# rhuangr/MARL-Maze

Measured on AMD Instinct MI355X. Metric: env-steps/sec (2-agent 10x10 maze) + PPO updates/sec, higher is better.
Workload: dtype f32; 1 GPU; PPO rollout+GAE+update over 65536 parallel 10x10 2-agent mazes per GPU (configs[2], the north-star workload: 65,536 parallel 10x10 mazes per GPU); mazes_per_gpu=65536, maze=10x10 (layout 19x19), horizon=16, global_batch=1048575, minibatch=209715, minibatch_steps_per_iter=25, parallelism=dp1, rollout=stream launches, gemm=x2, parity_mode=True

## Files before the change

include/marlmaze.h:

```cpp
#ifndef MARLMAZE_H
#define MARLMAZE_H

#include <stdint.h>

#ifdef __cplusplus
extern "C" {
#endif

#define MM_OBS_DIM 65
#define MM_MASK_DIM 6
#define MM_RNG_WORDS 625
#define MM_MAX_SIDE 41
#define MM_MAZES_PER_BLOCK 32

#define MM_E_ARG (-1)
#define MM_E_SIZE (-2)

#define MM_ST_GEN_FAIL 1u
#define MM_ST_BAD_MOVE 2u

typedef struct {
    int8_t x, y, dir, flags;
    int8_t lmx, lmy, olsx, olsy;
    int8_t minx, maxx, miny, maxy;
// ... 250 lines not shown
int mm_par_accum(const uint8_t* done, const float* reward, const int32_t* ep_stats, const int32_t* par, int n,
                 int quota, int32_t* counted, uint64_t* totals, void* stream);

#define MM_ELOG_WORDS 16
#define MM_ELOG_LEN 0
#define MM_ELOG_SHORTEST 1
#define MM_ELOG_SOLVED 2
#define MM_ELOG_PAR 3
#define MM_ELOG_T_KEY 4
#define MM_ELOG_FETCHER 5
#define MM_ELOG_T_KNOW0 6
#define MM_ELOG_T_KNOW1 7
#define MM_ELOG_T_READY 8
#define MM_ELOG_CELLS0 9
#define MM_ELOG_CELLS1 10
#define MM_ELOG_CELLS_BOTH 11
#define MM_ELOG_OPEN 12
#define MM_ELOG_MARKS0 13
#define MM_ELOG_MARKS1 14
#define MM_ELOG_STAYS 15
long mm_elog_state_words(int layout_stride);
int mm_elog_init(int32_t* log, int32_t* counted, int32_t* state, int n, int quota, long state_words, void* stream);
int mm_elog_start(const mm_env_t* env, const uint8_t* select, int32_t* state, long state_words, void* stream);
int mm_elog_step(const mm_env_t* env, const int8_t* actions, const uint8_t* done, const float* reward,
                 const int32_t* ep_stats, const int32_t* par, int quota, int32_t* counted, int32_t* state,
                 long state_words, int32_t* log, void* stream);

int mm_critic_value(const float* x, int ldx, int K0, int M, int H0, int H1, const float* w0, const float* b0,
                    const float* w1, const float* b1, const float* w2, const float* b2, float* v, void* stream);

int mm_critic_update_ok(int M, int K0, int ldx);
int mm_critic_update(const float* x, int ldx, int K0, int M, const float* rtg, const uint16_t* w0_tp, const float* b0,
                     const uint16_t* w1_tp, const uint16_t* w1t_tp, const float* b1, const uint16_t* w2_tp,
                     const float* w2, const float* b2, float* v, float* dv, float* h0, float* h1, float* dy1,
                     float* dy0, float* cs1, float* cs0, void* stream);

int mm_actor_front_ws_len(void);
int mm_actor_front_prep(const float* const* wproj, const float* const* bproj, const float* wq, const float* wk,
                        const float* wv, float* ws, void* stream);
int mm_actor_front_fwd(const float* ws, const float* x, int ldx, int B, int parity, float* h, void* stream);

#define MM_FRONT_FWD_ROW1 0
#define MM_FRONT_FWD_ROW2 1
#define MM_FRONT_FWD_MFMA 2
int mm_actor_front_fwd_ex(const float* ws, const float* x, int ldx, int B, int parity, float* h, int algo,
                          void* stream);

int mm_actor_front_grad_len(void);
int mm_actor_front_partial_len(void);
int mm_actor_front_bwd(const float* ws, const float* x, int ldx, int B, int parity, const float* dh, float* partial,
                       int grid, float* red, float* grad, void* stream);
#define MM_FRONT_BWD_MFMA 0
#define MM_FRONT_BWD_VALU 1
int mm_actor_front_bwd_ex(const float* ws, const float* x, int ldx, int B, int parity, const float* dh,
                          float* partial, int grid, float* red, float* grad, int algo, void* stream);
int mm_actor_front_bwd_grid(int B, int algo);
int mm_actor_front_bwd_to(const float* ws, const float* x, int ldx, int B, int parity, const float* dh,
                          float* partial, int grid, float* red, float* const* wproj_grad, float* const* bproj_grad,
                          float* wq_grad, float* wk_grad, float* wv_grad, int algo, void* stream);

#ifdef __cplusplus
}
#endif
#endif
```

marl-maze_amd/csrc/actor_front.hip:

```cpp
#include <hip/hip_runtime.h>
#include <math.h>
#include <stdint.h>

#include "marlmaze.h"

namespace mm {

#ifndef FRONT_P3_UNROLL
#define FRONT_P3_UNROLL 4
#endif
#ifndef FRONT_EF_UNROLL
#define FRONT_EF_UNROLL 2
#endif
#ifndef FRONT_EF_ROWS
#define FRONT_EF_ROWS 4
#endif

constexpr int kTok = 23;
constexpr int kEmb = 20;
constexpr int kKq = 10;
constexpr int kQkv = 2 * kKq + kEmb;
constexpr int kPin = 4;
constexpr int kRowF = kTok * kEmb;
constexpr float kSqrtKq = 3.16227766016838f;
// ... 1342 lines not shown
            for (int I = 0; I < 2; I++)
                if (16 * I + c16 < 24)
#pragma unroll
                    for (int J = 0; J < 2; J++)
                        t_store(T + (16 * I + c16) * kTp + 16 * J + 4 * q4, dS[J][I], t_sw(c16));
            wave_sync();
            f32x4_t dK[2] = {f32x4_t{0.f, 0.f, 0.f, 0.f}, f32x4_t{0.f, 0.f, 0.f, 0.f}};
            f32x4_t dQ[2] = {f32x4_t{0.f, 0.f, 0.f, 0.f}, f32x4_t{0.f, 0.f, 0.f, 0.f}};
#pragma unroll
            for (int s = 0; s < kKH; s++) {
                const int i = kh_row(s, q4);
#pragma unroll
                for (int J = 0; J < 2; J++) dK[J] = mfma4(T[i * kTp + 16 * J + t_col(s, c16, q4)], qb[s], dK[J]);
#pragma unroll
                for (int I = 0; I < 2; I++) {
                    const int rb = (16 * I + c16) * kTp;
                    const float tv = s < 4 ? T[(rb + 4 * q4 + t_sw(c16)) ^ s] : T[rb + 16 + 4 * (s - 4) + (q4 ^ t_sw(c16))];
                    dQ[I] = mfma4(ka[s], tv, dQ[I]);
                }
            }
            front_prio(2);
            wave_sync();
#pragma unroll
            for (int I = 0; I < 2; I++) {
                const int i = 16 * I + c16;
                if (i < kTok && q4 < 3)
                    *reinterpret_cast<float4*>(my + kMG + i * kQkv + 4 * q4) =
                        make_float4(dQ[I][0], dQ[I][1], dQ[I][2], dQ[I][3]);
            }
#pragma unroll
            for (int J = 0; J < 2; J++)
#pragma unroll
                for (int g = 0; g < 4; g++) {
                    const int j = 16 * J + 4 * q4 + g;
                    if (j < kTok) {
                        if (c16 < kKq) my[kMG + j * kQkv + kKq + c16] = dK[J][g];
#pragma unroll
                        for (int C = 0; C < 2; C++)
                            if (16 * C + c16 < kEmb) my[kMG + j * kQkv + 2 * kKq + 16 * C + c16] = dV[J][C][g];
                    }
                }
        }
        float4 fp[kEFPf];
        ef2_prefetch(dh + (size_t)row0 * kRowF, nrow, 0, fp);
        if (hs < nrow && tok < kTok) *reinterpret_cast<float4*>(sm + hs * kMSample + kMX + tok * kPin) = xv;
        __syncthreads();
#ifndef FRONT_DIAG_NO_EF
        ef2_accumulate<kMSample, kMG, kMX>(sm, dh + (size_t)row0 * kRowF, nrow, fp, ef);
#endif
    }
    ef2_write(partial, ef);
}

constexpr int kSumCols = 64, kSumClasses = 16;

__global__ __launch_bounds__(kSumCols * kSumClasses) void k_front_sum(const float* __restrict__ partial, int rows,
                                                                      double* __restrict__ red) {
    __shared__ double acc_s[kSumClasses][kSumCols];
    const int c = threadIdx.x % kSumCols, k = threadIdx.x / kSumCols;
    const int e = blockIdx.x * kSumCols + c;
    double acc = 0.0;
    if (e < kPartLen) {
        int r = k;
        for (; r + 7 * kSumClasses < rows; r += 8 * kSumClasses) {
            float v[8];
#pragma unroll
            for (int i = 0; i < 8; i++) v[i] = partial[(size_t)(r + i * kSumClasses) * kPartLen + e];
#pragma unroll
            for (int i = 0; i < 8; i++) acc += (double)v[i];
        }
        for (; r < rows; r += kSumClasses) acc += (double)partial[(size_t)r * kPartLen + e];
    }
    acc_s[k][c] = acc;
    __syncthreads();
    if (k == 0 && e < kPartLen) {
        double t = 0.0;
#pragma unroll
        for (int q = 0; q < kSumClasses; q++) t += acc_s[q][c];
        red[e] = t;
    }
}

struct FrontGradPtrs {
    float* wq;
    float* wk;
    float* wv;
    float* wp[kTok];
    float* bp[kTok];
};

template <bool SCATTER>
__global__ __launch_bounds__(256) void k_front_combine(const float* __restrict__ ws, const double* __restrict__ red,
                                                       float* __restrict__ grad, FrontGradPtrs dst) {
    const int e = blockIdx.x * blockDim.x + threadIdx.x;
    if (e >= kGradLen) return;
    auto put = [&](double vd) {
        const float v = (float)vd;
        if (!SCATTER) {
            grad[e] = v;
        } else if (e < kGP) {
            const int r = e / kEmb, c = e % kEmb;
            float* d = r < kKq ? dst.wq + r * kEmb : r < 2 * kKq ? dst.wk + (r - kKq) * kEmb : dst.wv + (r - 2 * kKq) * kEmb;
            d[c] = v;
        } else if (e < kGB) {
            const int f = e - kGP, tk = f / (kEmb * kPin), c = (f / kPin) % kEmb, k = f % kPin;
            if (k < c_dims[tk]) dst.wp[tk][c * c_dims[tk] + k] = v;
        } else {
            const int f = e - kGB;
            dst.bp[f / kEmb][f % kEmb] = v;
        }
    };
    const float* W = ws + kWsW;
    if (e < kGP) {
        const int r = e / kEmb, c = e % kEmb;
        double acc = 0.0;
        for (int tk = 0; tk < kTok; tk++) {
            const float* Wp = ws + kWsWP + (tk * kEmb + c) * kPin;
            const double* E = red + kPEF + (tk * kGd + r) * kPin;
#pragma unroll
            for (int a = 0; a < kPin; a++) acc = fma(E[a], (double)Wp[a], acc);
            acc = fma(red[kPef + tk * kGd + r], (double)ws[kWsBP + tk * kEmb + c], acc);
        }
        put(acc);
    } else if (e < kGB) {
        const int f = e - kGP, tk = f / (kEmb * kPin), c = (f / kPin) % kEmb, k = f % kPin;
        double acc = red[kPEF + (tk * kGd + kQkv + c) * kPin + k];
        for (int r = 0; r < kQkv; r++) acc = fma((double)W[r * kEmb + c], red[kPEF + (tk * kGd + r) * kPin + k], acc);
        put(acc);
    } else {
        const int f = e - kGB, tk = f / kEmb, c = f % kEmb;
        double acc = red[kPef + tk * kGd + kQkv + c];
        for (int r = 0; r < kQkv; r++) acc = fma((double)W[r * kEmb + c], red[kPef + tk * kGd + r], acc);
        put(acc);
    }
}

}

using namespace mm;

extern "C" int mm_actor_front_ws_len(void) { return kWsLen; }
extern "C" int mm_actor_front_grad_len(void) { return kGradLen; }
static int cu_count() {
    static int cus[64] = {0};
    int dev = 0;
    if (hipGetDevice(&dev) != hipSuccess || dev < 0 || dev >= 64) return 256;
    if (!cus[dev] && hipDeviceGetAttribute(&cus[dev], hipDeviceAttributeMultiprocessorCount, dev) != hipSuccess)
        cus[dev] = 256;
    return cus[dev];
}

extern "C" int mm_actor_front_partial_len(void) { return kPartLen; }

extern "C" int mm_actor_front_bwd_grid(int B, int algo) {
    if (B < 0 || (algo != MM_FRONT_BWD_MFMA && algo != MM_FRONT_BWD_VALU)) return MM_E_ARG;
    const int rows = algo == MM_FRONT_BWD_MFMA ? kMRows : kBwdRows;
    const int per_cu = algo == MM_FRONT_BWD_MFMA ? kMPerCU : 2;
    const int groups = (B + rows - 1) / rows;
    const int cap = per_cu * cu_count();
    return groups < 1 ? 1 : (groups < cap ? groups : cap);
}

extern "C" int mm_actor_front_prep(const float* const* wproj, const float* const* bproj, const float* wq,
                                   const float* wk, const float* wv, float* ws, void* stream) {
    if (!wproj || !bproj || !wq || !wk || !wv || !ws) return MM_E_ARG;
    ProjPtrs P;
    for (int i = 0; i < kTok; i++) {
        if (!wproj[i] || !bproj[i]) return MM_E_ARG;
        P.w[i] = wproj[i];
        P.b[i] = bproj[i];
    }
    hipLaunchKernelGGL(k_front_prep, dim3(kTok), dim3(256), 0, (hipStream_t)stream, P, wq, wk, wv, ws);
    return (int)hipGetLastError();
}


extern "C" int mm_actor_front_fwd_ex(const float* ws, const float* x, int ldx, int B, int parity, float* h,
                                     int algo, void* stream) {
    if (!ws || !x || !h || B < 0 || ldx < MM_OBS_DIM) return MM_E_ARG;
    if (algo != MM_FRONT_FWD_ROW1 && algo != MM_FRONT_FWD_ROW2 && algo != MM_FRONT_FWD_MFMA) return MM_E_ARG;
    if (B == 0) return 0;
    if (algo == MM_FRONT_FWD_MFMA) {
        const int groups = (B + kFMRows - 1) / kFMRows;
        const int cap = FRONT_FM_WAVES * cu_count();
        const int grid = groups < cap ? groups : cap;
        hipLaunchKernelGGL(k_front_fwd_mfma<false>, dim3(grid), dim3(256), 0, (hipStream_t)stream, ws, x, ldx, B,
                           parity, (void*)h);
    } else if (algo == MM_FRONT_FWD_ROW2) {
        const int groups = (B + kF2Rows - 1) / kF2Rows;
        const int grid = groups < 2 * cu_count() ? groups : 2 * cu_count();
        hipLaunchKernelGGL(k_front_fwd2, dim3(grid), dim3(256), 0, (hipStream_t)stream, ws, x, ldx, B, parity, h);
    } else {
        const int groups = (B + kFwdRows - 1) / kFwdRows;
        const int grid = groups < 3 * cu_count() ? groups : 3 * cu_count();
        hipLaunchKernelGGL(k_front_fwd<false>, dim3(grid), dim3(256), 0, (hipStream_t)stream, ws, x, ldx, B, parity,
                           (void*)h);
    }
    return (int)hipGetLastError();
}

extern "C" int mm_actor_front_fwd_h16_ex(const float* ws, const float* x, int ldx, int B, int parity, void* h,
                                         int algo, void* stream) {
    if (!ws || !x || !h || B < 0 || ldx < MM_OBS_DIM || ((uintptr_t)h & 7)) return MM_E_ARG;
    if (algo != MM_FRONT_FWD_ROW1 && algo != MM_FRONT_FWD_MFMA) return MM_E_ARG;
    if (B == 0) return 0;
    if (algo == MM_FRONT_FWD_MFMA) {
        const int groups = (B + kFMRows - 1) / kFMRows;
        const int cap = FRONT_FM_WAVES * cu_count();
        const int grid = groups < cap ? groups : cap;
        hipLaunchKernelGGL(k_front_fwd_mfma<true>, dim3(grid), dim3(256), 0, (hipStream_t)stream, ws, x, ldx, B,
                           parity, h);
    } else {
        const int groups = (B + kFwdRows - 1) / kFwdRows;
        const int grid = groups < 3 * cu_count() ? groups : 3 * cu_count();
        hipLaunchKernelGGL(k_front_fwd<true>, dim3(grid), dim3(256), 0, (hipStream_t)stream, ws, x, ldx, B, parity,
                           h);
    }
    return (int)hipGetLastError();
}

extern "C" int mm_actor_front_fwd_h16(const float* ws, const float* x, int ldx, int B, int parity, void* h,
                                      void* stream) {
    return mm_actor_front_fwd_h16_ex(ws, x, ldx, B, parity, h, MM_FRONT_FWD_ROW1, stream);
}

extern "C" int mm_actor_front_fwd(const float* ws, const float* x, int ldx, int B, int parity, float* h,
                                  void* stream) {
    return mm_actor_front_fwd_ex(ws, x, ldx, B, parity, h, MM_FRONT_FWD_ROW1, stream);
}

static int front_bwd(const float* ws, const float* x, int ldx, int B, int parity, const float* dh, float* partial,
                     int grid, float* red, float* grad, const FrontGradPtrs* dst, int algo, void* stream) {
    if (!ws || !x || !dh || !partial || !red || (!grad && !dst) || B < 0 || ldx < MM_OBS_DIM || grid <= 0)
        return MM_E_ARG;
    if ((uintptr_t)red & 7) return MM_E_ARG;
    if (algo != MM_FRONT_BWD_MFMA && algo != MM_FRONT_BWD_VALU) return MM_E_ARG;
    hipStream_t s = (hipStream_t)stream;
    double* red64 = reinterpret_cast<double*>(red);
    if (algo == MM_FRONT_BWD_MFMA)
        hipLaunchKernelGGL(k_front_bwd_mfma, dim3(grid), dim3(kMThreads), 0, s, ws, x, ldx, B, parity, dh, partial);
    else
        hipLaunchKernelGGL(k_front_bwd, dim3(grid), dim3(kBwdThreads), 0, s, ws, x, ldx, B, parity, dh, partial);
    hipError_t e = hipGetLastError();
    if (e != hipSuccess) return (int)e;
    hipLaunchKernelGGL(k_front_sum, dim3((kPartLen + kSumCols - 1) / kSumCols), dim3(kSumCols * kSumClasses), 0, s,
                       partial, grid, red64);
    e = hipGetLastError();
    if (e != hipSuccess) return (int)e;
    if (grad)
        hipLaunchKernelGGL(k_front_combine<false>, dim3((kGradLen + 255) / 256), dim3(256), 0, s, ws, red64, grad,
                           FrontGradPtrs{});
    else
        hipLaunchKernelGGL(k_front_combine<true>, dim3((kGradLen + 255) / 256), dim3(256), 0, s, ws, red64, nullptr, *dst);
    return (int)hipGetLastError();
}

extern "C" int mm_actor_front_bwd_ex(const float* ws, const float* x, int ldx, int B, int parity, const float* dh,
                                     float* partial, int grid, float* red, float* grad, int algo, void* stream) {
    if (!grad) return MM_E_ARG;
    return front_bwd(ws, x, ldx, B, parity, dh, partial, grid, red, grad, nullptr, algo, stream);
}

extern "C" int mm_actor_front_bwd_to(const float* ws, const float* x, int ldx, int B, int parity, const float* dh,
                                     float* partial, int grid, float* red, float* const* wproj_grad,
                                     float* const* bproj_grad, float* wq_grad, float* wk_grad, float* wv_grad,
                                     int algo, void* stream) {
    if (!wproj_grad || !bproj_grad || !wq_grad || !wk_grad || !wv_grad) return MM_E_ARG;
    FrontGradPtrs d;
    d.wq = wq_grad;
    d.wk = wk_grad;
    d.wv = wv_grad;
    for (int i = 0; i < kTok; i++) {
        if (!wproj_grad[i] || !bproj_grad[i]) return MM_E_ARG;
        d.wp[i] = wproj_grad[i];
        d.bp[i] = bproj_grad[i];
    }
    return front_bwd(ws, x, ldx, B, parity, dh, partial, grid, red, nullptr, &d, algo, stream);
}

extern "C" int mm_actor_front_bwd(const float* ws, const float* x, int ldx, int B, int parity, const float* dh,
                                  float* partial, int grid, float* red, float* grad, void* stream) {
    return mm_actor_front_bwd_ex(ws, x, ldx, B, parity, dh, partial, grid, red, grad, MM_FRONT_BWD_VALU, stream);
}
```

marl-maze_amd/marlmaze/_lib.py:

```python
import ctypes
import os

import torch

PKG_ROOT = os.path.dirname(os.path.dirname(os.path.abspath(__file__)))
LIB_PATH = os.environ.get("MARLMAZE_LIB") or os.path.join(PKG_ROOT, "libmarlmaze.so")

OBS_DIM = 65
MASK_DIM = 6
RNG_WORDS = 625
MAX_SIDE = 41
MAZES_PER_BLOCK = 32

ST_GEN_FAIL = 1
ST_BAD_MOVE = 2

GAE_AUTO, GAE_COLUMN, GAE_WALK, GAE_SCAN = 0, 1, 2, 3

ACT_SAMPLE, ACT_GREEDY = 0, 1
ACT_MODES = {"sample": ACT_SAMPLE, "greedy": ACT_GREEDY}

EVAL_WORDS = 32
EV_EPISODES, EV_SOLVED, EV_TIMEOUTS, EV_SUM_LEN, EV_SUM_LEN_SOLVED, EV_SUM_SHORT_SOLVED = 0, 1, 2, 3, 4, 5
EV_MIN_LEN_SOLVED, EV_MAX_LEN_SOLVED, EV_SUM_RATIO_Q16, EV_BAD_SHORT = 6, 7, 8, 9
EV_HIST0, EV_HIST_BINS = 16, 16

PAR_WORDS = 32
PAR_EPISODES, PAR_SUM_LEN, PAR_SUM_PAR, PAR_SUM_RATIO_Q16, PAR_AT_PAR, PAR_BELOW = 0, 1, 2, 3, 4, 5
PAR_UNRATED, PAR_MAX_EXCESS = 6, 7
PAR_HIST0, PAR_HIST_BINS = 16, 16

ELOG_WORDS = 16
ELOG_LEN, ELOG_SHORTEST, ELOG_SOLVED, ELOG_PAR, ELOG_T_KEY, ELOG_FETCHER, ELOG_T_KNOW0, ELOG_T_KNOW1 = range(8)
ELOG_T_READY, ELOG_CELLS0, ELOG_CELLS1, ELOG_CELLS_BOTH, ELOG_OPEN, ELOG_MARKS0, ELOG_MARKS1, ELOG_STAYS = range(8, 16)
ELOG_FIELDS = ("LEN", "SHORTEST", "SOLVED", "PAR", "T_KEY", "FETCHER", "T_KNOW0", "T_KNOW1", "T_READY", "CELLS0",
               "CELLS1", "CELLS_BOTH", "OPEN", "MARKS0", "MARKS1", "STAYS")

AF_KNOWS_END = 1
AF_SEES_END = 2
AF_OTHER_KNOWS = 4
AF_HAS_KEY = 8
AF_SEES_KEY = 16
AF_TEAM_KEY = 32
AF_HAS_MARK = 64

EXPORTS = ("mm_version", "mm_env_desc_size", "mm_layout_stride", "mm_env_seed", "mm_env_reset",
           "mm_env_step", "mm_env_step_timed", "mm_env_reset_done", "mm_env_pregen", "mm_gae", "mm_gae_ex", "mm_sample", "mm_head_sample", "mm_head_sample_ex", "mm_heads_fwd",
           "mm_actor_front_ws_len", "mm_actor_front_prep", "mm_actor_front_fwd", "mm_actor_front_fwd_ex",
           "mm_actor_front_grad_len", "mm_actor_front_partial_len", "mm_actor_front_bwd", "mm_actor_front_bwd_ex",
           "mm_actor_front_bwd_to", "mm_actor_front_bwd_grid",
           "mm_x3_tp_len", "mm_x3_tp_pack", "mm_x3_nt", "mm_x3_nt_f32a", "mm_x3_mbits_len",
           "mm_x3_heads_bwd", "mm_ppo_loss_partials", "mm_ppo_loss", "mm_ppo_loss_bwd",
           "mm_gemm_tp_len", "mm_gemm_tp_pack", "mm_gemm_nt", "mm_gemm_nt_algo", "mm_gemm_wgrad_algo", "mm_gemm_wgrad_ws_len",
           "mm_gemm_wgrad", "mm_colsum", "mm_mse_loss_partials", "mm_mse_loss", "mm_losses_final",
           "mm_clip_adam_ws_len", "mm_clip_adam", "mm_gemm_tp_pack_multi", "mm_gemm_wgrad_slices",
           "mm_gemm_wgrad_partials", "mm_colsum_multi_ws_len", "mm_colsum_multi", "mm_wsum_multi", "mm_critic_value",
           "mm_gemm_range_flag", "mm_gemm_nt_h", "mm_gemm_a16_ok", "mm_gemm_wgrad_h", "mm_gemm_wgrad_partials_h",
           "mm_heads_fwd_h16", "mm_x3_heads_bwd_h16", "mm_trunk3_ok", "mm_trunk3",
           "mm_trunk3_head_sample_ok", "mm_trunk3_head_sample", "mm_actor_front_fwd_h16",
           "mm_actor_front_fwd_h16_ex", "mm_head_act", "mm_act", "mm_eval_init", "mm_eval_accum",
           "mm_env_dist", "mm_env_par", "mm_par_init", "mm_par_accum",
           "mm_elog_state_words", "mm_elog_init", "mm_elog_start", "mm_elog_step",
           "mm_gemm_x2p_ok", "mm_x3_heads_bwd_x2p",
           "mm_critic_update_ok", "mm_critic_update")
VERSION = 308

PREC_X3, PREC_F16, PREC_X2 = 0, 1, 2
FRONT_BWD = {"mfma": 0, "valu": 1}
FRONT_FWD = {"row1": 0, "row2": 1, "mfma": 2}
GEMM_ALGO = {"auto": 0, "stream": 1}
GEMM_A_F16, GEMM_C_F16, GEMM_B_F16 = 1, 2, 4
GEMM_A_X2P, GEMM_C_X2P, GEMM_B_X2P = 8, 16, 32


class EnvDesc(ctypes.Structure):
    _fields_ = [
        ("n", ctypes.c_int32), ("size_w", ctypes.c_int32), ("size_h", ctypes.c_int32),
        ("max_timestep", ctypes.c_int32), ("difficulty", ctypes.c_int32),
        ("rand_start", ctypes.c_int32), ("rand_sizes", ctypes.c_int32),
        ("rand_lo", ctypes.c_int32), ("rand_hi", ctypes.c_int32),
        ("layout_stride", ctypes.c_int32),
        ("layout", ctypes.c_void_p), ("agents", ctypes.c_void_p), ("mazes", ctypes.c_void_p),
        ("rng", ctypes.c_void_p), ("work", ctypes.c_void_p),
        ("next_layout", ctypes.c_void_p), ("next_mazes", ctypes.c_void_p), ("next_rng", ctypes.c_void_p),
        ("gen_state", ctypes.c_void_p),
    ]


class AdamSeg(ctypes.Structure):
    _fields_ = [
        ("param", ctypes.c_void_p), ("grad", ctypes.c_void_p), ("exp_avg", ctypes.c_void_p),
        ("exp_avg_sq", ctypes.c_void_p), ("n", ctypes.c_long), ("max_norm", ctypes.c_float),
        ("step_size", ctypes.c_float), ("bc2_sqrt", ctypes.c_float), ("grad_scale", ctypes.c_float),
    ]


class PackSeg(ctypes.Structure):
    _fields_ = [("X", ctypes.c_void_p), ("R", ctypes.c_int), ("C", ctypes.c_int), ("ld", ctypes.c_int),
                ("trans", ctypes.c_int), ("tp", ctypes.c_void_p)]


class ColsumSeg(ctypes.Structure):
    _fields_ = [("x", ctypes.c_void_p), ("R", ctypes.c_long), ("N", ctypes.c_int), ("out", ctypes.c_void_p)]


class WsumSeg(ctypes.Structure):
    _fields_ = [("x", ctypes.c_void_p), ("n", ctypes.c_long), ("S", ctypes.c_int), ("out", ctypes.c_void_p)]


_LIB = None


class _Lib:

    def __init__(self, cdll):
        self._cdll = cdll

    def __getattr__(self, name):
        try:
            return getattr(self._cdll, name)
        except AttributeError:
# ... 237 lines not shown
```

marl-maze_amd/marlmaze/networks.py:

```python
import ctypes
import math
import os

import numpy as np
import torch
import torch.nn as nn
import torch.nn.functional as F

FEATURE_DIMS = [4, 4, 4, 4, 4, 4, 4, 4, 4, 4, 4, 4, 2, 2, 1, 4, 1, 1, 1, 1, 1, 1, 2]
FEATURE_AMOUNT = len(FEATURE_DIMS)
OBS_SPACE = int(np.sum(FEATURE_DIMS))
EMBEDDING_DIM = 20
KQ_DIM = 10
_SQRT_KQ = float(np.sqrt(KQ_DIM))


class Projection(nn.Module):

    def __init__(self, parity_mode=True):
        super().__init__()
        self.layers = nn.ModuleList([nn.Linear(d, EMBEDDING_DIM) for d in FEATURE_DIMS])
        self.parity_mode = parity_mode
        starts = np.zeros(FEATURE_AMOUNT, np.int64) if parity_mode else np.cumsum([0] + FEATURE_DIMS[:-1])
        self.register_buffer("_starts", torch.as_tensor(starts), persistent=False)
        self.in_width = 4 if parity_mode else OBS_SPACE

    def packed(self):
        rows = []
        for lin, d, s in zip(self.layers, FEATURE_DIMS, self._starts.tolist()):
            w = lin.weight
            left = s
            right = self.in_width - s - d
            rows.append(F.pad(w, (left, right)))
        return torch.cat(rows, 0), torch.cat([lin.bias for lin in self.layers], 0)

    def forward(self, x, packed=None):
        W, b = packed if packed is not None else self.packed()
        return F.linear(x[:, :self.in_width], W, b)


class m_Attention(nn.Module):

    def __init__(self, kq_dim=KQ_DIM):
        super().__init__()
        self.kq_dim = kq_dim
        self.keys = nn.Linear(EMBEDDING_DIM, kq_dim, bias=False)
        self.querys = nn.Linear(EMBEDDING_DIM, kq_dim, bias=False)
        self.values = nn.Linear(EMBEDDING_DIM, EMBEDDING_DIM, bias=False)

    def forward(self, h):
        B = h.shape[0]
        t = h.view(B, FEATURE_AMOUNT, EMBEDDING_DIM)
        wqkv = torch.cat([self.querys.weight, self.keys.weight, self.values.weight], 0)
        qkv = F.linear(t, wqkv)
        q, k, v = qkv.split([self.kq_dim, self.kq_dim, EMBEDDING_DIM], dim=-1)
        logits = torch.bmm(q, k.transpose(1, 2)) / _SQRT_KQ
        w = torch.softmax(logits, dim=-1)
        ctx = torch.bmm(w, v)
        return (t + ctx).reshape(B, FEATURE_AMOUNT * EMBEDDING_DIM)


_CUS = {}
FRONT_BWD_ALGO = os.environ.get("MARLMAZE_FRONT_BWD", "mfma")


def _front_bwd_grid(B, dev):
    from . import _lib

    with torch.cuda.device(dev):
        grid = _lib.lib().mm_actor_front_bwd_grid(int(B), _lib.FRONT_BWD[FRONT_BWD_ALGO])
    if grid < 1:
        raise _lib.MMError(f"mm_actor_front_bwd_grid failed with status {grid}")
    return grid
FRONT_FWD_ALGO = os.environ.get("MARLMAZE_FRONT_FWD", "mfma")
FRONT_FWD_ROW2_MAX = int(os.environ.get("MARLMAZE_FRONT_FWD_ROW2_MAX", "8192"))


def _cu_count(dev):
    if dev not in _CUS:
        _CUS[dev] = torch.cuda.get_device_properties(dev).multi_processor_count
    return _CUS[dev]


class _FusedFront(torch.autograd.Function):

    @staticmethod
    def forward(ctx, x, parity, *params):
        x = x.contiguous()
        ws, h = _front_fwd(x, parity, params)
        ctx.save_for_backward(x, ws)
        ctx.parity = parity
        return h

    @staticmethod
    def backward(ctx, dh):
        from . import _lib

        x, ws = ctx.saved_tensors
        B = x.shape[0]
        dh = dh.contiguous()
        L = _lib.lib()
        grid = _front_bwd_grid(B, x.device)
        plen = L.mm_actor_front_partial_len()
        partial = torch.empty((grid, plen), dtype=torch.float32, device=x.device)
        red = torch.empty(plen, dtype=torch.float64, device=x.device)
        g = torch.empty(L.mm_actor_front_grad_len(), dtype=torch.float32, device=x.device)
        _lib.check(L.mm_actor_front_bwd_ex(_lib.ptr(ws), _lib.ptr(x), OBS_SPACE, B, int(ctx.parity), _lib.ptr(dh),
                                           _lib.ptr(partial), grid, _lib.ptr(red), _lib.ptr(g),
                                           _lib.FRONT_BWD[FRONT_BWD_ALGO], _lib.stream_ptr()), "mm_actor_front_bwd_ex")
        n_qk, n_v = KQ_DIM * EMBEDDING_DIM, EMBEDDING_DIM * EMBEDDING_DIM
        dwq = g[0:n_qk].view(KQ_DIM, EMBEDDING_DIM)
        dwk = g[n_qk:2 * n_qk].view(KQ_DIM, EMBEDDING_DIM)
        dwv = g[2 * n_qk:2 * n_qk + n_v].view(EMBEDDING_DIM, EMBEDDING_DIM)
        o = 2 * n_qk + n_v
        n_p = FEATURE_AMOUNT * EMBEDDING_DIM * 4
        dwp = g[o:o + n_p].view(FEATURE_AMOUNT, EMBEDDING_DIM, 4)
        dbp = g[o + n_p:].view(FEATURE_AMOUNT, EMBEDDING_DIM)
        return (None, None, *(dwp[i, :, :d] for i, d in enumerate(FEATURE_DIMS)),
                *(dbp[i] for i in range(FEATURE_AMOUNT)), dwq, dwk, dwv)


def front_params(projection, attention):
    return ([lin.weight for lin in projection.layers] + [lin.bias for lin in projection.layers] +
            [attention.querys.weight, attention.keys.weight, attention.values.weight])


GEMM_PRECISIONS = ("x3", "x2", "f16")
FP32_GEMM = os.environ.get("MARLMAZE_FP32_GEMM", "x2")
if FP32_GEMM not in ("x2", "x3"):
    raise ValueError(f"MARLMAZE_FP32_GEMM must be 'x2' or 'x3', not {FP32_GEMM!r}")
_MAX_WIDTH = 272
_WARNED = set()


def _engine_ok(x, widths):
    return x.is_cuda and x.dim() == 2 and x.stride(1) == 1 and all(n <= _MAX_WIDTH for n in widths)


def _warn_torch_path(what):
    if what not in _WARNED:
        _WARNED.add(what)
        import warnings

        warnings.warn(f"marlmaze: {what} is outside the hand-written GEMM engine's shapes; it runs as plain "
                      "torch ops", RuntimeWarning, stacklevel=3)


def _grad_scale(M, prec):
    return float(2.0 ** int(math.floor(math.log2(max(int(M), 1))))) if prec in ("f16", "x2") else 1.0


def _wgrad(dy, x, prec, out=None, nk=None):
    from . import x3

    s = _grad_scale(dy.shape[0], prec)
    if x3.is_planes(dy):
        return x3.wgrad(dy, x, prec=prec, dscale=1.0, cscale=1.0 / s, out=out, nk=nk)
    if dy.dtype == torch.float16:
        return x3.wgrad(dy.contiguous(), x, prec=prec, dscale=1.0, cscale=1.0 / s, out=out)
    return x3.wgrad(dy.contiguous(), x, prec=prec, dscale=s, out=out)


# ... 357 lines not shown
            with torch.no_grad():
                hs, _ = _mlp_fwd(h, params[0::2], params[1::2], self.gemm_prec, False)
            return hs[-1]
        act = self.activation()
        for lin in self.layers:
            h = act(F.linear(h, lin.weight, lin.bias))
        return h

    def train_forward(self, x):
        x = x.contiguous()
        params = self._mlp_params()
        wl = [lin.weight for lin in self.layers]
        act16 = (_act16(self.gemm_prec, x.shape[0], [w_.shape[0] for w_ in wl],
                        [(w_.shape[0], w_.shape[1]) for w_ in wl[1:]]) and (wl[-1].shape[0] + 31) // 32 == 9)
        h16 = act16 and F16_H0 and wl[0].shape[1] % 4 == 0
        ws, h0 = _front_fwd(x, self.projection.parity_mode, front_params(self.projection, self.attention), h16=h16)
        if not self._engine(h0):
            raise ValueError("Actor.train_forward needs the GPU engine's shapes (ReLU, widths <= 272)")
        x2p = len(wl) > 1 and _x2p(self.gemm_prec, x.shape[0], [tuple(w_.shape) for w_ in wl[1:]])
        hs, bits = _mlp_fwd(h0, params[0::2], params[1::2], self.gemm_prec, True, act16=act16, x2p=x2p)
        w, b = self.heads()
        z = _heads_fwd(hs[-1], w, b)
        if x2p:
            from . import x3

            hs = [_SavedPlanes(h) if x3.is_planes(h) else h for h in hs]
        return z, (x, ws, hs, bits)

    def train_backward(self, saved, dz):
        x, ws, hs, bits = saved
        hs = [h.planes() if isinstance(h, _SavedPlanes) else h for h in hs]
        L = len(self.layers)
        w, _ = self.heads()
        gw = self._adjacent(_grad_of(self.move_head.weight), _grad_of(self.mark_head.weight))
        gb = self._adjacent(_grad_of(self.move_head.bias), _grad_of(self.mark_head.bias))
        params = self._mlp_params()
        g16 = _g16(self.gemm_prec, hs, params[0::2], True)
        from . import x3

        x2p = x3.is_planes(hs[L - 1])
        dy, cs, dwh, dbh = _heads_bwd(dz.contiguous(), hs[L], w, bits[L - 1], out_w=gw, out_b=gb,
                                      oscale=_grad_scale(dz.shape[0], self.gemm_prec) if g16 or x2p else None,
                                      x2p=x2p)
        if gw is None:
            self.move_head.weight.grad.copy_(dwh[:5])
            self.mark_head.weight.grad.copy_(dwh[5:])
        if gb is None:
            self.move_head.bias.grad.copy_(dbh[:5])
            self.mark_head.bias.grad.copy_(dbh[5:])
        params = self._mlp_params()
        dh0, _ = _mlp_bwd(bits, hs, params[0::2], dy, cs, self.gemm_prec, True,
                          outs=[_grad_of(p) for p in params])
        _front_bwd_to(ws, x, self.projection.parity_mode, dh0,
                      [_grad_of(p) for p in front_params(self.projection, self.attention)])


def _front_fwd_algo(B):
    if FRONT_FWD_ALGO == "auto":
        return "row2" if B <= FRONT_FWD_ROW2_MAX else "row1"
    return FRONT_FWD_ALGO


def _front_fwd(x, parity, params, h16=False):
    from . import _lib

    from . import x3

    L = _lib.lib()
    B = x.shape[0]
    stream = _lib.stream_ptr()

    def prep():
        ws = torch.empty(L.mm_actor_front_ws_len(), dtype=torch.float32, device=x.device)
        ptrs = [p.data_ptr() for p in params]
        wp = (ctypes.c_void_p * FEATURE_AMOUNT)(*ptrs[:FEATURE_AMOUNT])
        bp = (ctypes.c_void_p * FEATURE_AMOUNT)(*ptrs[FEATURE_AMOUNT:2 * FEATURE_AMOUNT])
        wq, wk, wv = params[2 * FEATURE_AMOUNT:]
        _lib.check(L.mm_actor_front_prep(wp, bp, _lib.ptr(wq), _lib.ptr(wk), _lib.ptr(wv), _lib.ptr(ws), stream),
                   "mm_actor_front_prep")
        return ws

    ws = x3.cached_value("front_prep", params, prep)
    if h16:
        h = torch.empty((B, FEATURE_AMOUNT * EMBEDDING_DIM), dtype=torch.float16, device=x.device)
        algo = _lib.FRONT_FWD["mfma" if _front_fwd_algo(B) == "mfma" else "row1"]
        _lib.check(L.mm_actor_front_fwd_h16_ex(_lib.ptr(ws), _lib.ptr(x), OBS_SPACE, B, int(parity), _lib.ptr(h),
                                               algo, stream), "mm_actor_front_fwd_h16_ex")
        return ws, h
    h = torch.empty((B, FEATURE_AMOUNT * EMBEDDING_DIM), dtype=torch.float32, device=x.device)
    _lib.check(L.mm_actor_front_fwd_ex(_lib.ptr(ws), _lib.ptr(x), OBS_SPACE, B, int(parity), _lib.ptr(h),
                                       _lib.FRONT_FWD[_front_fwd_algo(B)], stream), "mm_actor_front_fwd_ex")
    return ws, h


def _front_bwd_to(ws, x, parity, dh, grads):
    from . import _lib

    L = _lib.lib()
    B = x.shape[0]
    dh = dh.contiguous()
    grid = _front_bwd_grid(B, x.device)
    plen = L.mm_actor_front_partial_len()
    partial = torch.empty((grid, plen), dtype=torch.float32, device=x.device)
    red = torch.empty(plen, dtype=torch.float64, device=x.device)
    assert all(g.is_contiguous() for g in grads)
    ptrs = [g.data_ptr() for g in grads]
    gw = (ctypes.c_void_p * FEATURE_AMOUNT)(*ptrs[:FEATURE_AMOUNT])
    gb = (ctypes.c_void_p * FEATURE_AMOUNT)(*ptrs[FEATURE_AMOUNT:2 * FEATURE_AMOUNT])
    gq, gk, gv = grads[2 * FEATURE_AMOUNT:]
    _lib.check(L.mm_actor_front_bwd_to(_lib.ptr(ws), _lib.ptr(x), OBS_SPACE, B, int(parity), _lib.ptr(dh),
                                       _lib.ptr(partial), grid, _lib.ptr(red), gw, gb, _lib.ptr(gq), _lib.ptr(gk),
                                       _lib.ptr(gv), _lib.FRONT_BWD[FRONT_BWD_ALGO], _lib.stream_ptr()),
               "mm_actor_front_bwd_to")


class Critic(nn.Module):

    def __init__(self, agent_amount, hidden_sizes=(128, 128), activation=nn.ReLU, gemm_prec=None):
        super().__init__()
        hidden_sizes = list(hidden_sizes)
        gemm_prec = FP32_GEMM if gemm_prec is None else gemm_prec
        assert gemm_prec in GEMM_PRECISIONS
        self.gemm_prec = gemm_prec
        self.layers = nn.ModuleList()
        self.activation = activation
        self.agent_amount = agent_amount
        self.layers.append(nn.Linear(agent_amount * OBS_SPACE, hidden_sizes[0]))
        for a, b in zip(hidden_sizes[:-1], hidden_sizes[1:]):
            self.layers.append(nn.Linear(a, b))
        self.layers.append(nn.Linear(hidden_sizes[-1], 1))
        self.initialize_weights()

    def initialize_weights(self):
        for layer in self.layers:
            nn.init.orthogonal_(layer.weight)

    def _params(self):
        return [t for lin in self.layers for t in (lin.weight, lin.bias)]

    def _engine(self, x):
        ok = (len(self.layers) == 3 and self.activation is nn.ReLU and x.shape[1] % 2 == 0
              and all(lin.weight.shape[0] <= 64 for lin in self.layers)
              and _engine_ok(x, [lin.weight.shape[0] for lin in self.layers]))
        if x.is_cuda and not ok:
            _warn_torch_path("this Critic")
        return ok

    def forward(self, x):
        x = torch.as_tensor(x, dtype=torch.float32, device=self.layers[0].weight.device)
        x = x.reshape(-1, self.agent_amount * OBS_SPACE)
        if self._engine(x):
            x = x.contiguous()
            params = self._params()
            if torch.is_grad_enabled() and any(p.requires_grad for p in params):
                return _EngineCritic.apply(self.gemm_prec, x, *params)
            with torch.no_grad():
                return _critic_fwd(x, params, self.gemm_prec, False)[0]
        act = self.activation()
        for lin in self.layers[:-1]:
            x = act(F.linear(x, lin.weight, lin.bias))
        return F.linear(x, self.layers[-1].weight, self.layers[-1].bias)

    @torch.no_grad()
    def value_into(self, x, out):
        from . import _lib
# ... 75 lines not shown
```

Before: 7.458 million env-steps/s.

## Add split-fp16 x2 MFMA attention backward kernel, auto-selected for x2 GEMM precision

Adds a new attention backward kernel that computes the dP and dV products with 16x16x32 fp16 MFMAs on hi/lo split operands. The incoming gradient is scaled by a per-wave power-of-two exponent so the split keeps precision. The f32 4-wide MFMAs are kept for the S, dK and dQ products. The kernel is selected automatically when the actor's GEMM precision is x2, replacing the previous mfma default in that path. The aim is fewer, denser matrix instructions in the backward pass, at the cost of extra conversion work, more LDS traffic and slightly different numerics.

```diff
diff --git a/include/marlmaze.h b/include/marlmaze.h
--- a/include/marlmaze.h
+++ b/include/marlmaze.h
@@ -326,6 +326,7 @@
                        int grid, float* red, float* grad, void* stream);
 #define MM_FRONT_BWD_MFMA 0
 #define MM_FRONT_BWD_VALU 1
+#define MM_FRONT_BWD_X2 2
 int mm_actor_front_bwd_ex(const float* ws, const float* x, int ldx, int B, int parity, const float* dh,
                           float* partial, int grid, float* red, float* grad, int algo, void* stream);
 int mm_actor_front_bwd_grid(int B, int algo);
diff --git a/marl-maze_amd/csrc/actor_front.hip b/marl-maze_amd/csrc/actor_front.hip
--- a/marl-maze_amd/csrc/actor_front.hip
+++ b/marl-maze_amd/csrc/actor_front.hip
@@ -1418,6 +1418,328 @@
     ef2_write(partial, ef);
 }
 
+constexpr int kXDh = 0, kXDl = kXDh + kTok * kEmb;
+constexpr int kXPp = 24;
+constexpr int kXPh = kXDl + kTok * kEmb, kXPl = kXPh + 24 * kXPp;
+constexpr int kXSample = 1040;
+constexpr int kXZero = 16;
+static_assert(kXPl + 24 * kXPp + 8 <= 2 * kXSample, "the fp16 images (and a block's overrun) live in the sample's region");
+static_assert(kMSample <= kXSample && (kXSample * 4) % 16 == 0, "QKV, T and G | x live in the sample's region");
+static_assert(kXPh % 4 == 0 && kXPl % 4 == 0 && kXDl % 4 == 0, "8-byte aligned images");
+constexpr int kXTarget = 14;
+
+__device__ __forceinline__ f32x4_t mfma16h(fm_f16x8 a, fm_f16x8 b, f32x4_t c) {
+    return __builtin_amdgcn_mfma_f32_16x16x32_f16(a, b, c, 0, 0, 0);
+}
+
+__device__ __forceinline__ uint32_t wave_umax(uint32_t v) {
+    v = max(v, (uint32_t)__builtin_amdgcn_mov_dpp((int)v, 0xB1, 0xF, 0xF, true));
+    v = max(v, (uint32_t)__builtin_amdgcn_mov_dpp((int)v, 0x4E, 0xF, 0xF, true));
+    v = max(v, (uint32_t)__builtin_amdgcn_mov_dpp((int)v, 0x141, 0xF, 0xF, true));
+    v = max(v, (uint32_t)__builtin_amdgcn_mov_dpp((int)v, 0x140, 0xF, 0xF, true));
+    const auto a = __builtin_amdgcn_permlane16_swap(v, v, false, false);
+    v = max(a[0], a[1]);
+    const auto b = __builtin_amdgcn_permlane32_swap(v, v, false, false);
+    return max(b[0], b[1]);
+}
+
+__device__ __forceinline__ uint32_t abs_bits(float4 v) {
+    const uint32_t m = 0x7fffffffu;
+    return max(max(__float_as_uint(v.x) & m, __float_as_uint(v.y) & m),
+               max(__float_as_uint(v.z) & m, __float_as_uint(v.w) & m));
+}
+
+__device__ __forceinline__ void x2_scale(uint32_t m, float& s, float& inv) {
+    const uint32_t e = m >> 23;
+    uint32_t se = min(127u + kXTarget + 127u - e, 253u);
+    if (e == 0u || e == 255u) se = 127u;
+    s = __uint_as_float(se << 23);
+    inv = __uint_as_float((254u - se) << 23);
+}
+
+__device__ __forceinline__ fm_f16x8 x2_row8(const uint16_t* p0, const uint16_t* p1) {
+    const uint2 a = *reinterpret_cast<const uint2*>(p0), b = *reinterpret_cast<const uint2*>(p1);
+    return __builtin_bit_cast(fm_f16x8, make_uint4(a.x, a.y, b.x, b.y));
+}
+__device__ __forceinline__ fm_f16x8 x2_col8(const uint16_t* p, int o4) {
+    const fm_s4 a = fm_tr(p), b = fm_tr(p + o4);
+    return __builtin_bit_cast(fm_f16x8, __builtin_shufflevector(a, b, 0, 1, 2, 3, 4, 5, 6, 7));
+}
+
+__device__ __forceinline__ void softmax_ds(f32x4_t (&S)[2][2], f32x4_t (&dP)[2][2], int c16, int q4, float back) {
+#pragma unroll
+    for (int I = 0; I < 2; I++) {
+        float mx = -INFINITY;
+#pragma unroll
+        for (int J = 0; J < 2; J++)
+#pragma unroll
+            for (int g = 0; g < 4; g++)
+                if (16 * J + 4 * q4 + g < kTok) mx = fmaxf(mx, S[J][I][g]);
+        mx = xq_max(mx);
+        float sum = 0.f;
+#pragma unroll
+        for (int J = 0; J < 2; J++)
+#pragma unroll
+            for (int g = 0; g < 4; g++) {
+                float e = __builtin_amdgcn_exp2f((S[J][I][g] - mx) * kLog2eRsqrtKq);
+                e = 16 * J + 4 * q4 + g < kTok ? e : 0.f;
+                S[J][I][g] = e;
+                sum += e;
+            }
+        const float inv = 16 * I + c16 < kTok ? __builtin_amdgcn_rcpf(xq_sum(sum)) : 0.f;
+        float rs = 0.f;
+#pragma unroll
+        for (int J = 0; J < 2; J++)
+#pragma unroll
+            for (int g = 0; g < 4; g++) {
+                const float p = S[J][I][g] * inv;
+                S[J][I][g] = p;
+                rs = fmaf(dP[J][I][g], p, rs);
+            }
+        rs = xq_sum(rs);
+#pragma unroll
+        for (int J = 0; J < 2; J++)
+#pragma unroll
+            for (int g = 0; g < 4; g++) dP[J][I][g] = (S[J][I][g] * (dP[J][I][g] - rs)) * (kRSqrtKq * back);
+    }
+}
+
+__global__ __launch_bounds__(kMThreads) __attribute__((amdgpu_waves_per_eu(3))) void k_front_bwd_x2(const float* __restrict__ ws,
+                                                                   const float* __restrict__ x, int ldx, int B,
+                                                                   int parity, const float* __restrict__ dh,
+                                                                   float* __restrict__ partial) {
+    static_assert(kMRows == 8, "k_front_bwd_x2 is built for 8-sample workgroups");
+    __shared__ __attribute__((aligned(16))) float sm[kMRows * kXSample + kXZero];
+    __shared__ __attribute__((aligned(16))) float tab[kTok * kTabS];
+    const int wave = threadIdx.x >> 6;
+    for (int e = threadIdx.x; e < kMRows * kXSample + kXZero; e += kMThreads) sm[e] = 0.f;
+    for (int e = threadIdx.x; e < kTok * (kQkv * kPin + kQkv); e += kMThreads) {
+        const int t = e / (kQkv * kPin + kQkv), f = e % (kQkv * kPin + kQkv);
+        tab[t * kTabS + f] = f < kQkv * kPin ? ws[kWsAT + t * kQkv * kPin + f] : ws[kWsC + t * kQkv + f - kQkv * kPin];
+    }
+    EFAccM ef;
+    ef2_zero(ef);
+    const int iters = (B + kMRows - 1) / kMRows;
+    const int tok = threadIdx.x & 31, hs = 2 * wave + ((threadIdx.x >> 5) & 1);
+    const uint16_t* zero = reinterpret_cast<const uint16_t*>(sm + kMRows * kXSample);
+    for (int it = blockIdx.x; it < iters; it += gridDim.x) {
+        const int row0 = it * kMRows;
+        const int nrow = min(kMRows, B - row0);
+        __syncthreads();
+        float4 xv = make_float4(0.f, 0.f, 0.f, 0.f);
+        if (hs < nrow && tok < kTok) {
+            xv = xslice(x + (size_t)(row0 + hs) * ldx, tok, parity != 0);
+            float o[kQkv];
+            affine4t<kQkv>(tab + tok * kTabS, tab + tok * kTabS + kQkv * kPin, xv, o);
+            float2* q2 = reinterpret_cast<float2*>(sm + hs * kXSample + tok * kQp);
+            q2[0] = make_float2(o[0], o[1]), q2[1] = make_float2(o[2], o[3]);
+            q2[2] = make_float2(o[4], o[5]), q2[3] = make_float2(o[6], o[7]);
+            q2[4] = make_float2(o[8], o[9]), q2[5] = make_float2(0.f, 0.f);
+            q2[6] = make_float2(o[10], o[11]), q2[7] = make_float2(o[12], o[13]);
+            q2[8] = make_float2(o[14], o[15]), q2[9] = make_float2(o[16], o[17]);
+            q2[10] = make_float2(o[18], o[19]), q2[11] = make_float2(0.f, 0.f);
+            uint2* v2 = reinterpret_cast<uint2*>(q2 + kVO / 2);
+            uint32_t vh[kEmb / 2], vl[kEmb / 2];
+#pragma unroll
+            for (int k = 0; k < kEmb / 2; k++) fm_pair2(o[2 * kKq + 2 * k], o[2 * kKq + 2 * k + 1], kFMVs, vh[k], vl[k]);
+#pragma unroll
+            for (int k = 0; k < kEmb / 4; k++) {
+                v2[k] = make_uint2(vh[2 * k], vh[2 * k + 1]);
+                v2[kEmb / 4 + k] = make_uint2(vl[2 * k], vl[2 * k + 1]);
+            }
+        }
+        wave_sync();
+#pragma unroll 1
+        for (int half = 0; half < 2; half++) {
+            const int slot = 2 * wave + half;
+            if (slot >= nrow) break;
+            int lane = threadIdx.x & 63;
+            asm volatile("" : "+v"(lane));
+            const int c16 = lane & 15, q4 = (lane >> 4) & 3;
+            float* my = sm + slot * kXSample;
+            const float* QKV = my;
+            uint16_t* img = reinterpret_cast<uint16_t*>(my);
+            const float4* dh4 = reinterpret_cast<const float4*>(dh + (size_t)(row0 + slot) * kRowF);
+            const float4 d0 = dh4[lane];
+            float4 d1 = dh4[min(lane + 64, kRowF / 4 - 1)];
+            if (lane + 64 >= kRowF / 4) d1 = make_float4(0.f, 0.f, 0.f, 0.f);
+            float sd, sdi;
+            x2_scale(wave_umax(max(abs_bits(d0), abs_bits(d1))), sd, sdi);
+            front_prio(0);
+            f32x4_t S[2][2];
+            {
+                float kf[2][3], qf[2][3];
+#pragma unroll
+                for (int t = 0; t < 2; t++)
+#pragma unroll
+                    for (int e = 0; e < 3; e++) {
+                        const int r = min(16 * t + c16, kTok - 1);
+                        kf[t][e] = QKV[r * kQp + kKO + 4 * e + q4];
+                        qf[t][e] = QKV[r * kQp + kQO + 4 * e + q4];
+                    }
+#pragma unroll
+                for (int J = 0; J < 2; J++)
+#pragma unroll
+                    for (int I = 0; I < 2; I++) {
+                        f32x4_t acc = f32x4_t{0.f, 0.f, 0.f, 0.f};
+#pragma unroll
+                        for (int e = 0; e < 3; e++) acc = mfma4(kf[J][e], qf[I][e], acc);
+                        S[J][I] = acc;
+                    }
+            }
+            fm_f16x8 vah[2], val[2];
+#pragma unroll
+            for (int J = 0; J < 2; J++) {
+                const uint16_t* vr = img + min(16 * J + c16, kTok - 1) * (2 * kQp) + 2 * kVO + 8 * q4;
+                vah[J] = x2_row8(q4 < 3 ? vr : zero, q4 < 2 ? vr + 4 : zero);
+                val[J] = x2_row8(q4 < 3 ? vr + kEmb : zero, q4 < 2 ? vr + kEmb + 4 : zero);
+            }
+            float qb[kKH], ka[kKH];
+            {
+                const int ca = min(c16, kKq);
+#pragma unroll
+                for (int s = 0; s < kKH; s++) {
+                    const int r = kh_row(s, q4);
+                    qb[s] = QKV[min(r, kTok - 1) * kQp + kQO + ca];
+                    ka[s] = r < kTok ? QKV[min(r, kTok - 1) * kQp + kKO + ca] : 0.f;
+                }
+            }
+            wave_sync();
+            {
+                uint2* ih = reinterpret_cast<uint2*>(img + kXDh);
+                uint2* il = reinterpret_cast<uint2*>(img + kXDl);
+                uint32_t h0, h1, l0, l1;
+                fm_pair2(d0.x, d0.y, sd, h0, l0);
+                fm_pair2(d0.z, d0.w, sd, h1, l1);
+                ih[lane] = make_uint2(h0, h1), il[lane] = make_uint2(l0, l1);
+                fm_pair2(d1.x, d1.y, sd, h0, l0);
+                fm_pair2(d1.z, d1.w, sd, h1, l1);
+                if (lane + 64 < kRowF / 4) ih[lane + 64] = make_uint2(h0, h1), il[lane + 64] = make_uint2(l0, l1);
+            }
+            wave_sync();
+            f32x4_t dP[2][2];
+            {
+                fm_f16x8 dbh[2], dbl[2];
+#pragma unroll
+                for (int I = 0; I < 2; I++) {
+                    const uint16_t* dr = img + kXDh + min(16 * I + c16, kTok - 1) * kEmb + 8 * q4;
+                    dbh[I] = x2_row8(q4 < 3 ? dr : zero, q4 < 2 ? dr + 4 : zero);
+                    dbl[I] = x2_row8(q4 < 3 ? dr + (kXDl - kXDh) : zero, q4 < 2 ? dr + (kXDl - kXDh) + 4 : zero);
+                }
+                const f32x4_t z = f32x4_t{0.f, 0.f, 0.f, 0.f};
+#pragma unroll
+                for (int J = 0; J < 2; J++)
+#pragma unroll
+                    for (int I = 0; I < 2; I++) {
+                        f32x4_t accx = mfma16h(vah[J], dbl[I], z);
+                        accx = mfma16h(val[J], dbh[I], accx);
+                        const f32x4_t acc = mfma16h(vah[J], dbh[I], z);
+#pragma unroll
+                        for (int g = 0; g < 4; g++) dP[J][I][g] = fmaf(accx[g], kFMLoInv, acc[g]);
+                    }
+            }
+            front_prio(1);
+            softmax_ds(S, dP, c16, q4, kFMVsInv * sdi);
+            f32x4_t (&P)[2][2] = S;
+            f32x4_t (&dS)[2][2] = dP;
+#pragma unroll
+            for (int I = 0; I < 2; I++)
+#pragma unroll
+                for (int J = 0; J < 2; J++) {
+                    uint32_t h0, h1, l0, l1;
+                    fm_pair2(P[J][I][0], P[J][I][1], 1.f, h0, l0);
+                    fm_pair2(P[J][I][2], P[J][I][3], 1.f, h1, l1);
+                    if (16 * I + c16 < 24 && 16 * J + 4 * q4 < 24) {
+                        uint16_t* pw = img + kXPh + (16 * I + c16) * kXPp + 16 * J + 4 * q4;
+                        *reinterpret_cast<uint2*>(pw) = make_uint2(h0, h1);
+                        *reinterpret_cast<uint2*>(pw + (kXPl - kXPh)) = make_uint2(l0, l1);
+                    }
+                }
+            front_prio(0);
+            wave_sync();
+            f32x4_t dV[2][2];
+            {
+                const int tq = (lane >> 2) & 3, tp = lane & 3;
+                const bool in = q4 < 3;
+                const uint16_t* pb = in ? img + kXPh + (8 * q4 + tq) * kXPp + 4 * tp : zero;
+                const uint16_t* db = in ? img + kXDh + (8 * q4 + tq) * kEmb + 4 * tp : zero;
+                const int po4 = in ? 4 * kXPp : 0, do4 = in ? 4 * kEmb : 0;
+                const int pj = in ? 16 : 0;
+                const int pl = in ? kXPl - kXPh : 0, dl = in ? kXDl - kXDh : 0;
+                fm_f16x8 pah[2], pal[2], dbh[2], dbl[2];
+#pragma unroll
+                for (int t = 0; t < 2; t++) {
+                    pah[t] = x2_col8(pb + t * pj, po4);
+                    pal[t] = x2_col8(pb + t * pj + pl, po4);
+                    dbh[t] = x2_col8(db + t * pj, do4);
+                    dbl[t] = x2_col8(db + t * pj + dl, do4);
+                }
+                const f32x4_t z = f32x4_t{0.f, 0.f, 0.f, 0.f};
+#pragma unroll
+                for (int J = 0; J < 2; J++)
+#pragma unroll
+                    for (int C = 0; C < 2; C++) {
+                        f32x4_t accx = mfma16h(pah[J], dbl[C], z);
+                        accx = mfma16h(pal[J], dbh[C], accx);
+                        const f32x4_t acc = mfma16h(pah[J], dbh[C], z);
+#pragma unroll
+                        for (int g = 0; g < 4; g++) dV[J][C][g] = fmaf(accx[g], kFMLoInv, acc[g]) * sdi;
+                    }
+            }
+            wave_sync();
+            float* T = my;
+#pragma unroll
+            for (int I = 0; I < 2; I++)
+                if (16 * I + c16 < 24)
+#pragma unroll
+                    for (int J = 0; J < 2; J++)
+                        t_store(T + (16 * I + c16) * kTp + 16 * J + 4 * q4, dS[J][I], 0);
+            wave_sync();
+            f32x4_t dK[2] = {f32x4_t{0.f, 0.f, 0.f, 0.f}, f32x4_t{0.f, 0.f, 0.f, 0.f}};
+            f32x4_t dQ[2] = {f32x4_t{0.f, 0.f, 0.f, 0.f}, f32x4_t{0.f, 0.f, 0.f, 0.f}};
+#pragma unroll
+            for (int s = 0; s < kKH; s++) {
+                const int i = kh_row(s, q4);
+#pragma unroll
+                for (int J = 0; J < 2; J++) dK[J] = mfma4(T[i * kTp + 16 * J + c16], qb[s], dK[J]);
+#pragma unroll
+                for (int I = 0; I < 2; I++) {
+                    const int rb = min(16 * I + c16, 23) * kTp;
+                    const float tv = s < 4 ? T[rb + 4 * q4 + s] : T[rb + 16 + 4 * (s - 4) + q4];
+                    dQ[I] = mfma4(ka[s], tv, dQ[I]);
+                }
+            }
+            front_prio(2);
+            wave_sync();
+#pragma unroll
+            for (int I = 0; I < 2; I++) {
+                const int i = 16 * I + c16;
+                if (i < kTok && q4 < 3)
+                    *reinterpret_cast<float4*>(my + kMG + i * kQkv + 4 * q4) =
+                        make_float4(dQ[I][0], dQ[I][1], dQ[I][2], dQ[I][3]);
+            }
+#pragma unroll
+            for (int J = 0; J < 2; J++)
+#pragma unroll
+                for (int g = 0; g < 4; g++) {
+                    const int j = 16 * J + 4 * q4 + g;
+                    if (j < kTok) {
+                        if (c16 < kKq) my[kMG + j * kQkv + kKq + c16] = dK[J][g];
+#pragma unroll
+                        for (int C = 0; C < 2; C++)
+                            if (16 * C + c16 < kEmb) my[kMG + j * kQkv + 2 * kKq + 16 * C + c16] = dV[J][C][g];
+                    }
+                }
+        }
+        float4 fp[kEFPf];
+        ef2_prefetch(dh + (size_t)row0 * kRowF, nrow, 0, fp);
+        if (hs < nrow && tok < kTok) *reinterpret_cast<float4*>(sm + hs * kXSample + kMX + tok * kPin) = xv;
+        __syncthreads();
+        ef2_accumulate<kXSample, kMG, kMX>(sm, dh + (size_t)row0 * kRowF, nrow, fp, ef);
+    }
+    ef2_write(partial, ef);
+}
+
 constexpr int kSumCols = 64, kSumClasses = 16;
 
 __global__ __launch_bounds__(kSumCols * kSumClasses) void k_front_sum(const float* __restrict__ partial, int rows,
@@ -1519,9 +1841,9 @@
 extern "C" int mm_actor_front_partial_len(void) { return kPartLen; }
 
 extern "C" int mm_actor_front_bwd_grid(int B, int algo) {
-    if (B < 0 || (algo != MM_FRONT_BWD_MFMA && algo != MM_FRONT_BWD_VALU)) return MM_E_ARG;
-    const int rows = algo == MM_FRONT_BWD_MFMA ? kMRows : kBwdRows;
-    const int per_cu = algo == MM_FRONT_BWD_MFMA ? kMPerCU : 2;
+    if (B < 0 || (algo != MM_FRONT_BWD_MFMA && algo != MM_FRONT_BWD_VALU && algo != MM_FRONT_BWD_X2)) return MM_E_ARG;
+    const int rows = algo == MM_FRONT_BWD_VALU ? kBwdRows : kMRows;
+    const int per_cu = algo == MM_FRONT_BWD_VALU ? 2 : kMPerCU;
     const int groups = (B + rows - 1) / rows;
     const int cap = per_cu * cu_count();
     return groups < 1 ? 1 : (groups < cap ? groups : cap);
@@ -1600,11 +1922,13 @@
     if (!ws || !x || !dh || !partial || !red || (!grad && !dst) || B < 0 || ldx < MM_OBS_DIM || grid <= 0)
         return MM_E_ARG;
     if ((uintptr_t)red & 7) return MM_E_ARG;
-    if (algo != MM_FRONT_BWD_MFMA && algo != MM_FRONT_BWD_VALU) return MM_E_ARG;
+    if (algo != MM_FRONT_BWD_MFMA && algo != MM_FRONT_BWD_VALU && algo != MM_FRONT_BWD_X2) return MM_E_ARG;
     hipStream_t s = (hipStream_t)stream;
     double* red64 = reinterpret_cast<double*>(red);
     if (algo == MM_FRONT_BWD_MFMA)
         hipLaunchKernelGGL(k_front_bwd_mfma, dim3(grid), dim3(kMThreads), 0, s, ws, x, ldx, B, parity, dh, partial);
+    else if (algo == MM_FRONT_BWD_X2)
+        hipLaunchKernelGGL(k_front_bwd_x2, dim3(grid), dim3(kMThreads), 0, s, ws, x, ldx, B, parity, dh, partial);
     else
         hipLaunchKernelGGL(k_front_bwd, dim3(grid), dim3(kBwdThreads), 0, s, ws, x, ldx, B, parity, dh, partial);
     hipError_t e = hipGetLastError();
diff --git a/marl-maze_amd/marlmaze/_lib.py b/marl-maze_amd/marlmaze/_lib.py
--- a/marl-maze_amd/marlmaze/_lib.py
+++ b/marl-maze_amd/marlmaze/_lib.py
@@ -66,7 +66,7 @@
 VERSION = 308
 
 PREC_X3, PREC_F16, PREC_X2 = 0, 1, 2
-FRONT_BWD = {"mfma": 0, "valu": 1}
+FRONT_BWD = {"mfma": 0, "valu": 1, "x2": 2}
 FRONT_FWD = {"row1": 0, "row2": 1, "mfma": 2}
 GEMM_ALGO = {"auto": 0, "stream": 1}
 GEMM_A_F16, GEMM_C_F16, GEMM_B_F16 = 1, 2, 4
diff --git a/marl-maze_amd/marlmaze/networks.py b/marl-maze_amd/marlmaze/networks.py
--- a/marl-maze_amd/marlmaze/networks.py
+++ b/marl-maze_amd/marlmaze/networks.py
@@ -61,14 +61,24 @@
 
 
 _CUS = {}
-FRONT_BWD_ALGO = os.environ.get("MARLMAZE_FRONT_BWD", "mfma")
-
-
-def _front_bwd_grid(B, dev):
+FRONT_BWD_ALGO = os.environ.get("MARLMAZE_FRONT_BWD", "auto")
+
+
+def _front_bwd_algo(prec=None):
     from . import _lib
 
+    if FRONT_BWD_ALGO == "auto":
+        return "x2" if prec == "x2" else "mfma"
+    if FRONT_BWD_ALGO not in _lib.FRONT_BWD:
+        raise ValueError(f"FRONT_BWD_ALGO is {FRONT_BWD_ALGO!r}: one of auto, {', '.join(_lib.FRONT_BWD)}")
+    return FRONT_BWD_ALGO
+
+
+def _front_bwd_grid(B, dev, algo):
+    from . import _lib
+
     with torch.cuda.device(dev):
-        grid = _lib.lib().mm_actor_front_bwd_grid(int(B), _lib.FRONT_BWD[FRONT_BWD_ALGO])
+        grid = _lib.lib().mm_actor_front_bwd_grid(int(B), _lib.FRONT_BWD[algo])
     if grid < 1:
         raise _lib.MMError(f"mm_actor_front_bwd_grid failed with status {grid}")
     return grid
@@ -100,14 +110,15 @@
         B = x.shape[0]
         dh = dh.contiguous()
         L = _lib.lib()
-        grid = _front_bwd_grid(B, x.device)
+        algo = _front_bwd_algo()
+        grid = _front_bwd_grid(B, x.device, algo)
         plen = L.mm_actor_front_partial_len()
         partial = torch.empty((grid, plen), dtype=torch.float32, device=x.device)
         red = torch.empty(plen, dtype=torch.float64, device=x.device)
         g = torch.empty(L.mm_actor_front_grad_len(), dtype=torch.float32, device=x.device)
         _lib.check(L.mm_actor_front_bwd_ex(_lib.ptr(ws), _lib.ptr(x), OBS_SPACE, B, int(ctx.parity), _lib.ptr(dh),
                                            _lib.ptr(partial), grid, _lib.ptr(red), _lib.ptr(g),
-                                           _lib.FRONT_BWD[FRONT_BWD_ALGO], _lib.stream_ptr()), "mm_actor_front_bwd_ex")
+                                           _lib.FRONT_BWD[algo], _lib.stream_ptr()), "mm_actor_front_bwd_ex")
         n_qk, n_v = KQ_DIM * EMBEDDING_DIM, EMBEDDING_DIM * EMBEDDING_DIM
         dwq = g[0:n_qk].view(KQ_DIM, EMBEDDING_DIM)
         dwk = g[n_qk:2 * n_qk].view(KQ_DIM, EMBEDDING_DIM)
@@ -571,7 +582,7 @@
         dh0, _ = _mlp_bwd(bits, hs, params[0::2], dy, cs, self.gemm_prec, True,
                           outs=[_grad_of(p) for p in params])
         _front_bwd_to(ws, x, self.projection.parity_mode, dh0,
-                      [_grad_of(p) for p in front_params(self.projection, self.attention)])
+                      [_grad_of(p) for p in front_params(self.projection, self.attention)], prec=self.gemm_prec)
 
 
 def _front_fwd_algo(B):
@@ -612,13 +623,14 @@
     return ws, h
 
 
-def _front_bwd_to(ws, x, parity, dh, grads):
+def _front_bwd_to(ws, x, parity, dh, grads, prec=None):
     from . import _lib
 
     L = _lib.lib()
     B = x.shape[0]
     dh = dh.contiguous()
-    grid = _front_bwd_grid(B, x.device)
+    algo = _front_bwd_algo(prec)
+    grid = _front_bwd_grid(B, x.device, algo)
     plen = L.mm_actor_front_partial_len()
     partial = torch.empty((grid, plen), dtype=torch.float32, device=x.device)
     red = torch.empty(plen, dtype=torch.float64, device=x.device)
@@ -629,7 +641,7 @@
     gq, gk, gv = grads[2 * FEATURE_AMOUNT:]
     _lib.check(L.mm_actor_front_bwd_to(_lib.ptr(ws), _lib.ptr(x), OBS_SPACE, B, int(parity), _lib.ptr(dh),
                                        _lib.ptr(partial), grid, _lib.ptr(red), gw, gb, _lib.ptr(gq), _lib.ptr(gk),
-                                       _lib.ptr(gv), _lib.FRONT_BWD[FRONT_BWD_ALGO], _lib.stream_ptr()),
+                                       _lib.ptr(gv), _lib.FRONT_BWD[algo], _lib.stream_ptr()),
                "mm_actor_front_bwd_to")
 
 
```

New measurement: 7.522 million env-steps/s (median of 6 runs). Within noise of the previous version (+0.9%).
